# i3drobotics/i3dr_stereo_camera-ros

Measured on AMD Instinct MI355X. Metric: stereo pairs/sec + ms/frame, 1920×1080 D=256 8-path SGM, 1/2/4/8 MI355X, higher is better.
Workload: dtype u8

## Files before the change

i3dr_stereo_camera-ros_amd/csrc/census_sgm.hip:

```cpp
#include "sgm_device.h"

#include <atomic>
#include <string>

#ifndef SGM_WPE
#define SGM_WPE 4
#endif
#ifndef SGM_WPE32
#define SGM_WPE32 4
#endif
#ifndef SGM_NT_STORE
#define SGM_NT_STORE 1
#endif
#ifndef SGM_NT_LOAD
#define SGM_NT_LOAD 1
#endif
#ifndef SGM_EXP
#define SGM_EXP 0
#endif
#if SGM_EXP != 0 && !defined(SGM_EXPERIMENT_BUILD)
#error "SGM_EXP builds give invalid results: define SGM_EXPERIMENT_BUILD as well (never in a release build)"
#endif
#ifndef SGM_LRPRIO_HW
#define SGM_LRPRIO_HW 37
#endif
#ifndef SGM_LRPRIO_DIAG
#define SGM_LRPRIO_DIAG 64
#endif
#ifndef SGM_UPWTA_PRIO
#define SGM_UPWTA_PRIO 0
#endif
#ifndef SGM_ROWS_LPL8
#define SGM_ROWS_LPL8 0
#endif
#ifndef SGM_P32
#define SGM_P32 1
#endif

#include <algorithm>
#include <cstdio>
#include <cstdlib>
#include <vector>

namespace sgm {

#define SGM_CENSUS_BIT(B)                                                              \
    asm("v_cmp_lt_u32_sdwa vcc, %1, %2 src0_sel:BYTE_" #B " src1_sel:DWORD\n\t"      \
        "v_addc_co_u32_e32 %0, vcc, %0, %0, vcc"                                       \
        : "+v"(acc) : "v"(w), "v"(c) : "vcc")
__device__ __forceinline__ void census_bit(uint32_t& acc, uint32_t w, uint32_t c, int b)
{
    switch (b) {
    case 0: SGM_CENSUS_BIT(0); break;
    case 1: SGM_CENSUS_BIT(1); break;
    case 2: SGM_CENSUS_BIT(2); break;
    default: SGM_CENSUS_BIT(3); break;
    }
}
#undef SGM_CENSUS_BIT

template <int PITCH>
__device__ __forceinline__ uint64_t census_code_lds(const uint8_t* tile, int ty, int tx)
{
    static_assert(PITCH % 4 == 0, "u32 rows");
    const uint32_t* t32 = (const uint32_t*)tile + (PITCH / 4) * ty + (tx >> 2);
    const int sb = tx & 3;
    const uint32_t c = tile[(ty + 3) * PITCH + tx + 4];
    uint32_t lo = 0, hi = 0;
#pragma unroll
    for (int dy = 6; dy >= 0; dy--) {
        const uint32_t* r = t32 + (PITCH / 4) * dy;
        const uint32_t w0 = r[0], w1 = r[1], w2 = r[2];
        const uint32_t a0 = __builtin_amdgcn_alignbyte(w1, w0, sb);
        const uint32_t a1 = __builtin_amdgcn_alignbyte(w2, w1, sb);
        const uint32_t a2 = __builtin_amdgcn_alignbyte(w2, w2, sb);
#pragma unroll
        for (int dx = 8; dx >= 0; dx--) {
            if (dy == 3 && dx == 4) continue;
            const int k = dy * 9 + dx - (dy * 9 + dx > 31 ? 1 : 0);
            const uint32_t w = dx < 4 ? a0 : dx < 8 ? a1 : a2;
            if (k >= 32) census_bit(hi, w, c, dx & 3);
            else census_bit(lo, w, c, dx & 3);
        }
    }
    return (uint64_t)lo | ((uint64_t)hi << 32);
}

__global__ __launch_bounds__(256) void k_census9x7(const uint8_t* __restrict__ L, const uint8_t* __restrict__ R,
                                                   size_t stride, int W, int H,
                                                   uint64_t* __restrict__ cL, uint64_t* __restrict__ cR)
{
    __shared__ __attribute__((aligned(16))) uint8_t tile[10 * 72];
    const uint8_t* img = blockIdx.z ? R : L;
    uint64_t* out = blockIdx.z ? cR : cL;
    const int x0 = blockIdx.x * 64, y0 = blockIdx.y * 4;
    for (int i = threadIdx.x; i < 10 * 72; i += 256) {
        int ty = i / 72, tx = i - ty * 72;
        int yy = min(max(y0 + ty - 3, 0), H - 1), xx = min(max(x0 + tx - 4, 0), W - 1);
        tile[i] = img[(size_t)yy * stride + xx];
    }
    __syncthreads();
    const int tx = threadIdx.x & 63, ty = threadIdx.x >> 6;
    const int x = x0 + tx, y = y0 + ty;
    if (x >= W || y >= H) return;
    out[(size_t)y * W + x] = census_code_lds<72>(tile, ty, tx);
}

template <int DPL>
__device__ __forceinline__ void wload(const uint8_t* src, uint32_t (&wd)[(DPL + 3) / 4])
{
    if constexpr (DPL == 2) { wd[0] = *(const uint16_t*)src; }
    else if constexpr (DPL == 4) { wd[0] = *(const uint32_t*)src; }
    else if constexpr (DPL == 8) { const uint2 v = *(const uint2*)src; wd[0] = v.x; wd[1] = v.y; }
    else {
#pragma unroll
        for (int q = 0; q < DPL / 16; q++) {
// ... 245 lines not shown
    static constexpr int NPAD = LPL >= 16 ? NSEG + NSEG / 16 + 1 : NSEG + 4 * (NSEG / 32) + 4;
    static constexpr int NTOT = NSEG + NL;
    static constexpr int NLOAD = (NTOT + kWG - 1) / kWG;
    static constexpr int BUF = NPAD + NL + kWG;
    static __device__ __forceinline__ int phys(int e) { return LPL >= 16 ? e + (e >> 4) : e + 4 * (e >> 5); }
};
template <int DPL16>
struct RowsCfg {
#if SGM_ROWS_LPL8
    static constexpr int LPL = DPL16 <= 16 ? 8 : LineCfg<DPL16>::LPL;
#else
    static constexpr int LPL = LineCfg<DPL16>::LPL;
#endif
    static constexpr int DPL = DPL16 * 16 / LPL;
    static constexpr int NL = kWG / LPL;
};

template <int DPL, int LPL>
using SegRegs = uint64_t[RowSeg<DPL, LPL>::NLOAD];
template <int DPL, int LPL>
struct SegAddr {
    uint32_t off[RowSeg<DPL, LPL>::NLOAD];
    const char* lo;
};
template <int DPL, int LPL>
__device__ __forceinline__ SegAddr<DPL, LPL> seg_addr(const uint64_t* cL, const uint64_t* cR, const Geom& g, int tid)
{
    using RS = RowSeg<DPL, LPL>;
    SegAddr<DPL, LPL> a;
    const uint64_t* base = cL < cR ? cL : cR;
    const int bias = LPL * DPL + max(g.minD, 0);
    a.lo = (const char*)base - (size_t)8 * bias;
#pragma unroll
    for (int m = 0; m < RS::NLOAD; m++) {
        const int q = min(tid + m * kWG, RS::NTOT - 1);
        const int rel = q < RS::NSEG ? (int)(cR - base) + q - g.minD - LPL * DPL + 1 : (int)(cL - base) + (q - RS::NSEG);
        a.off[m] = (uint32_t)(8 * (rel + bias));
    }
    return a;
}
template <int DPL, int LPL>
__device__ __forceinline__ void seg_load(SegRegs<DPL, LPL>& v, const SegAddr<DPL, LPL>& a,
                                         const Geom& g, int rx, int ry, int xb, int s)
{
    const int y = ry > 0 ? s : g.H - 1 - s;
    const int yc = (SGM_EXP & 1) ? 0 : min(max(y, 0), g.H - 1);
    const char* sb = a.lo + (size_t)8 * ((size_t)yc * g.W + (xb + rx * s));
#pragma unroll
    for (int m = 0; m < RowSeg<DPL, LPL>::NLOAD; m++) v[m] = *(const uint64_t*)(sb + a.off[m]);
}

template <int DPL, int LPL>
__device__ __forceinline__ void seg_store(uint64_t* buf, const SegRegs<DPL, LPL>& v, int tid)
{
    using RS = RowSeg<DPL, LPL>;
#pragma unroll
    for (int m = 0; m < RS::NLOAD; m++) {
        const int q0 = tid + m * kWG;
        const int at = q0 < RS::NSEG ? RS::phys(q0) : (q0 < RS::NTOT ? RS::NPAD + (q0 - RS::NSEG) : RS::NPAD + RS::NL + tid);
        buf[at] = v[m];
    }
}

template <int DPL, bool EXACT, int LPL>
__device__ __forceinline__ void p16_seed(const uint8_t* src, const uint32_t (&imask)[DPL / 2], uint32_t (&Lr)[DPL / 2])
{
    uint32_t wd[(DPL + 3) / 4], Labs[DPL / 2];
    wload<DPL>(src, wd);
#pragma unroll
    for (int i = 0; i < DPL / 2; i++) {
        const uint32_t pr = __builtin_amdgcn_perm(0u, wd[i / 2], (i & 1) ? 0x0c030c02u : 0x0c010c00u);
        Labs[i] = pr | kBaseP2;
        if (!EXACT) Labs[i] = pk_max(Labs[i], imask[i]);
    }
    p16_relative<DPL, LPL>(Labs, Lr);
}

struct UpWta {
    const uint8_t* vols;
    size_t vol_bytes;
    uint64_t* res;
};
struct WtaPix { int best, minS, d16; bool rej; };
template <int DPL, bool EXACT>
__device__ __forceinline__ WtaPix wta_pix16(const uint32_t (&E)[(DPL + 3) / 4], const uint32_t (&O)[(DPL + 3) / 4],
                                            int p, const Geom& g, float inv_u, uint32_t* srow);
template <int DPL, bool EXACT>
__device__ __forceinline__ void wta_emask(int p, const Geom& g, uint32_t (&emaskE)[(DPL + 3) / 4],
                                          uint32_t (&emaskO)[(DPL + 3) / 4]);
template <int DPL>
__host__ __device__ constexpr size_t upwta_lds_bytes() { return (size_t)8 * 2 * RowSeg<DPL, 16>::BUF + (size_t)16 * 32 * ((DPL + 3) / 4) * 4; }

template <int DPL, bool EXACT, int LPL, bool FUSE = false, bool PRIO = false, int NP = 8>
__device__ __forceinline__ void p16_rows(const uint64_t* __restrict__ cL, const uint64_t* __restrict__ cR,
                                         uint8_t* __restrict__ V, uint8_t* __restrict__ trash, const Geom& g, int dir,
                                         int xb, const PathLaunch16& pl, uint64_t* lds, const UpWta& uw = UpWta{})
{
    static_assert(!FUSE || LPL == 16, "up+WTA blocks use 16 lanes per line (the WTA layout)");
    using RS = RowSeg<DPL, LPL>;
    constexpr int M = DPL / 2;
    constexpr int NL = RS::NL;
    const int tid = threadIdx.x;
    const int lane = tid & 63, w = tid >> 6;
    const int r = lane >> 4;
    const int p = LPL == 32 ? lane & 31 : LPL == 16 ? lane & 15 : (lane & 15) >> 1;
    const int j = LPL == 32 ? 2 * w + (lane >> 5) : LPL == 16 ? 4 * w + r : 8 * w + 2 * r + (lane & 1);
    const int rx = dir_rx(dir), ry = dir_ry(dir);
    int s0, s1;
    if (rx == 0) { s0 = 0; s1 = g.H; }
    else if (rx > 0) { s0 = max(0, g.minX1 - xb - (NL - 1)); s1 = min(g.H, g.maxX1 - xb); }
    else { s0 = max(0, xb - g.maxX1 + 1); s1 = min(g.H, xb + NL - g.minX1); }
    if (s0 >= s1) return;
    uint32_t imask[M], start[M];
    make_imask<DPL, EXACT, LPL>(p, g.D, imask, start);
    const uint32_t P1P1 = (uint32_t)g.P1 * 0x10001u, P2P2 = ((uint32_t)g.P2 + kBaseP) * 0x10001u;
    uint32_t Lr[M];
#pragma unroll
    for (int i = 0; i < M; i++) Lr[i] = start[i];
    bool pv = false;
    const uint8_t* bnd = pl.bnd[ry > 0 ? 0 : 1];
    if (bnd && s0 == 0) {
        const int x = xb + j, xp = x - rx;
        const bool cont = x >= g.minX1 && x < g.maxX1 && xp >= g.minX1 && xp < g.maxX1;
        const int xs = min(max(xp, g.minX1), g.maxX1 - 1) - g.minX1;
        uint32_t Ls[M];
        p16_seed<DPL, EXACT, LPL>(bnd + bnd_slot_of(dir) * pl.bnd_slot + (size_t)xs * g.D + p * DPL, imask, Ls);
#pragma unroll
        for (int i = 0; i < M; i++) Lr[i] = cont ? Ls[i] : Lr[i];
        pv = cont;
    }
    const bool lane_act = EXACT || p * DPL < g.D;
    const bool hi_ok = EXACT || p * DPL + 16 < g.D;
    uint8_t* const tr = trash + (tid & 63) * DPL;
    const int e_hi = j + (LPL - p) * DPL - 1;

    uint64_t* buf0 = lds;
    uint64_t* buf1 = lds + RS::BUF;
    uint64_t R0[RS::NLOAD], R1[RS::NLOAD], R2[RS::NLOAD], R3[RS::NLOAD];
    const SegAddr<DPL, LPL> sa = seg_addr<DPL, LPL>(cL, cR, g, tid);
    seg_load<DPL, LPL>(R0, sa, g, rx, ry, xb, s0);
    seg_store<DPL, LPL>(buf0, R0, tid);
    seg_load<DPL, LPL>(R1, sa, g, rx, ry, xb, min(s0 + 1, s1 - 1));
    seg_load<DPL, LPL>(R2, sa, g, rx, ry, xb, min(s0 + 2, s1 - 1));
    seg_load<DPL, LPL>(R3, sa, g, rx, ry, xb, min(s0 + 3, s1 - 1));
    __syncthreads();

    constexpr int NWD = (DPL + 3) / 4;
    constexpr int NV = NP - 1;
    uint32_t vw[NV][NWD], emaskE[NWD], emaskO[NWD];
    uint32_t* srow = (uint32_t*)(lds + 2 * RS::BUF) + j * 32 * NWD;
    const float inv_u = 1.0f / (float)max(100 - g.uniq, 1);
    const uint32_t voff = (uint32_t)((min(max(xb + j, g.minX1), g.maxX1 - 1) - g.minX1) * g.D + (lane_act ? p * DPL : 0));
    uint64_t vols0 = (uint64_t)uw.vols;
    if constexpr (FUSE) asm volatile("" : "+s"(vols0));
    auto vload = [&](int s) {
        const uint8_t* rb = (const uint8_t*)vols0 + (size_t)max(g.H - 1 - s, 0) * g.width1 * g.D;
#pragma unroll
        for (int k = 0; k < NV; k++) wload_buf<DPL>(rb + (size_t)(k == 0 ? 0 : k + 1) * uw.vol_bytes, voff, vw[k]);
    };
    if constexpr (FUSE) {
        wta_emask<DPL, EXACT>(p, g, emaskE, emaskO);
        vload(s0);
    }
    const uint64_t* resrow = FUSE ? uw.res + (size_t)(g.H - 1 - s0) * g.W : nullptr;
    auto step = [&](int s, const uint64_t* bufc) {
        const int x = xb + j + rx * s;
        const bool valid = s < s1 && x >= g.minX1 && x < g.maxX1;
        const int y = ry > 0 ? s : g.H - 1 - s;
        const uint64_t cl = bufc[RS::NPAD + j];
        uint32_t Labs[M];
        uint32_t E[NWD], O[NWD];
        if constexpr (FUSE) {
#pragma unroll
            for (int jj = 0; jj < NWD; jj++) {
                uint32_t e = 0, o = 0;
#pragma unroll
                for (int k = 0; k < NV; k++) {
                    e += vw[k][jj] & 0x00FF00FFu;
                    o += __builtin_amdgcn_perm(0u, vw[k][jj], 0x0c030c01u);
                }
                asm("" : "+v"(e), "+v"(o));
                E[jj] = e;
                O[jj] = o;
            }
        }
        const uint32_t P2x = pv ? P2P2 : kBaseP2;
        if constexpr (FUSE) __builtin_amdgcn_sched_barrier(0);
        p16_step<DPL, EXACT, LPL>(Lr, cl, [&](int k) { return bufc[RS::phys(e_hi - k)]; }, P1P1, P2x, imask, Labs);
        if constexpr (FUSE) {
            __builtin_amdgcn_sched_barrier(0);
#pragma unroll
            for (int jj = 0; jj < NWD; jj++) {
                const uint32_t a = Labs[2 * jj], b = 2 * jj + 1 < M ? Labs[2 * jj + 1] : 0u;
                E[jj] = (E[jj] + __builtin_amdgcn_perm(b, a, 0x0c040c00u)) | emaskE[jj];
                O[jj] = (O[jj] + __builtin_amdgcn_perm(b, a, 0x0c060c02u)) | emaskO[jj];
            }
            vload(s + 1);
            __builtin_amdgcn_sched_barrier(0);
            const WtaPix px = wta_pix16<DPL, EXACT>(E, O, p, g, inv_u, srow);
            const uint64_t v = (uint64_t)(uint16_t)(px.rej ? g.invalid : px.d16) |
                               ((uint64_t)(uint16_t)(px.rej ? -1 : px.best) << 16) | ((uint64_t)(uint16_t)px.minS << 32);
            const __amdgpu_buffer_rsrc_t rr = __builtin_amdgcn_make_buffer_rsrc((void*)resrow, 0, g.W * 8, 0x00020000);
            resrow -= g.W;
            typedef unsigned int v2u __attribute__((ext_vector_type(2)));
            __builtin_amdgcn_raw_buffer_store_b64(__builtin_bit_cast(v2u, v), rr,
                                                  (valid && p == 0) ? (uint32_t)x * 8u : 0x80000000u, 0, 2);
        } else {
            const bool ok = valid && lane_act && !((SGM_EXP & 2) && dir == 1);
            uint8_t* const vrow = V + (size_t)min(max(y, 0), g.H - 1) * g.width1 * g.D;
            uint8_t* const dst = ok ? vrow + (uint32_t)((x - g.minX1) * g.D + p * DPL) : tr;
            store_pairs<DPL>(dst, (ok && hi_ok) ? dst + 16 : tr + 16, Labs);
        }
        pv = valid;
    };
    auto body = [&](int s, const uint64_t* bcur, uint64_t* bnext, uint64_t (&Rnext)[RS::NLOAD],
                    uint64_t (&Rfree)[RS::NLOAD]) {
        seg_load<DPL, LPL>(Rfree, sa, g, rx, ry, xb, min(s + 4, s1 - 1));
        step(s, bcur);
        seg_store<DPL, LPL>(bnext, Rnext, tid);
        __syncthreads();
    };
    for (int s = s0; s < s1; s += 4) {
        if constexpr (PRIO) lr_prio(rx != 0 ? ((s1 - s) * SGM_LRPRIO_DIAG) >> 6 : s1 - s, g.H);
        body(s, buf0, buf1, R1, R0);
        body(s + 1, buf1, buf0, R2, R1);
        body(s + 2, buf0, buf1, R3, R2);
        body(s + 3, buf1, buf0, R0, R3);
    }
}

template <int DPL>
__host__ __device__ constexpr int rows_lds_codes() { return 2 * RowSeg<RowsCfg<DPL>::DPL, RowsCfg<DPL>::LPL>::BUF; }

template <int DPL, bool EXACT, bool PRIO = false, int NP = 0>
__device__ __forceinline__ void paths_block16(const PathFrames& pf, size_t vol_bytes, size_t trash_off,
                                              const Geom& g, const PathLaunch16& pl, uint32_t it, uint64_t* lds)
{
    using RC = RowsCfg<DPL>;
    using HC = LineCfg<DPL>;
    const int dir = (int)(it >> 24);
    const int f = (int)((it >> 22) & 3u);
    const int lb = (int)(it & 0x3FFFFFu);
    if (f >= pf.n || ((pf.skip_dirs >> dir) & 1u)) return;
    const uint64_t* cL = pick4(pf.cL, f);
    const uint64_t* cR = pick4(pf.cR, f);
    uint8_t* V = pick4(pf.vols, f) + (size_t)vol_slot(NP ? NP : pf.np, dir) * vol_bytes;
    uint8_t* trash = V + trash_off;
    const int y0 = lb * HC::HROWS + (64 / HC::LPL) * (threadIdx.x >> 6);
    if (dir == 6) p16_horiz<HC::DPL, EXACT, 1, PRIO, HC::LPL>(cL, cR, V, trash, g, y0);
    else if (dir == 7) p16_horiz<HC::DPL, EXACT, -1, PRIO, HC::LPL>(cL, cR, V, trash, g, y0);
    else p16_rows<RC::DPL, EXACT, RC::LPL, false, PRIO>(cL, cR, V, trash, g, dir, pl.xb_lo[dir] + lb * RC::NL, pl, lds);
}

__device__ __forceinline__ void trace_record(uint64_t* trace, uint64_t tag, uint64_t t0)
{
    const uint64_t t1 = __builtin_amdgcn_s_memrealtime();
    const uint32_t hw = __builtin_amdgcn_s_getreg((4 << 0) | (0 << 6) | (31 << 11));
    const uint32_t xcc = __builtin_amdgcn_s_getreg((20 << 0) | (0 << 6) | (15 << 11));
    uint64_t* r = trace + ((size_t)blockIdx.x * 4 + (threadIdx.x >> 6)) * 4;
    r[0] = tag | ((uint64_t)blockIdx.x << 32); r[1] = ((uint64_t)xcc << 32) | hw; r[2] = t0; r[3] = t1;
}

template <int DPL, bool EXACT>
__global__ __launch_bounds__(kWG) __attribute__((amdgpu_waves_per_eu(DPL >= 32 && !SGM_P32 ? SGM_WPE32 : SGM_WPE)))
void k_census_paths16(PathFrames pf, size_t vol_bytes, size_t trash_off, Geom g, PathLaunch16 pl,
                      const uint32_t* __restrict__ items, uint64_t* __restrict__ trace)
{
    __shared__ uint64_t lds[rows_lds_codes<DPL>()];
    const uint64_t t0 = trace ? __builtin_amdgcn_s_memrealtime() : 0;
    paths_block16<DPL, EXACT, true>(pf, vol_bytes, trash_off, g, pl, items[blockIdx.x], lds);
    if (trace && (threadIdx.x & 63) == 0)
        trace_record(trace, items[blockIdx.x], t0);
}

template <int DPL>
__host__ __device__ constexpr size_t wta_key_bytes(int W)
{
    return (size_t)kWG * 8 * ((DPL + 3) / 4) > (size_t)4 * W ? (size_t)kWG * 8 * ((DPL + 3) / 4) : (size_t)4 * W;
}
template <int DPL>
__host__ __device__ constexpr size_t wta_lds_bytes(int W) { return wta_key_bytes<DPL>(W) + RowLds::rest_bytes(W); }

template <int DPL, bool EXACT>
__device__ __forceinline__ WtaPix wta_pix16(const uint32_t (&E)[(DPL + 3) / 4], const uint32_t (&O)[(DPL + 3) / 4],
                                            int p, const Geom& g, float inv_u, uint32_t* srow)
{
    constexpr int NWD = (DPL + 3) / 4;
    constexpr int KB = DPL > 16 ? 5 : 4;
    constexpr uint32_t KMASK = (1u << KB) - 1;
    constexpr int G = pair_group(DPL);
    auto kof = [](int b) { return (uint32_t)(b < DPL ? vol_byte_d(G, b) : b) & KMASK; };
    uint32_t km = 0xFFFFFFFFu;
#pragma unroll
    for (int j = 0; j < NWD; j++) {
        uint32_t ce = (kof(4 * j + 2) << 16) | kof(4 * j), co = (kof(4 * j + 3) << 16) | kof(4 * j + 1);
        uint32_t ke, ko;
        if constexpr (EXACT && DPL >= 4) {
            asm("" : "+s"(ce), "+s"(co));
            ke = (E[j] << KB) | ce; ko = (O[j] << KB) | co;
        }
        else { ke = pk_shl(E[j], KB) | ce; ko = pk_shl(O[j], KB) | co; }
        km = pk_min(km, pk_min(ke, ko));
    }
    km = pk_min(km, alignbit16(km, km)) & 0xFFFFu;
    const uint32_t kmin = row_min_u32(((km >> KB) << 9) | (uint32_t)(p * DPL + (int)(km & KMASK)));
    WtaPix r;
    const int best = (int)(kmin & 511u);
    const int minS = (int)(kmin >> 9);
#pragma unroll
    for (int j = 0; j < NWD; j++) { srow[p * 2 * NWD + j] = E[j]; srow[p * 2 * NWD + NWD + j] = O[j]; }
    auto s_at = [&](int d) {
        const int kk = vol_d_byte(G, d % DPL);
        const uint32_t v = srow[(d / DPL) * 2 * NWD + (kk & 1) * NWD + (kk >> 2)];
        return (int)((v >> (16 * ((kk >> 1) & 1))) & 0xFFFFu);
    };
    const int sm = s_at(max(best - 1, 0)), sp = s_at(min(best + 1, 16 * DPL - 1));
    int T = 0;
    if (g.uniq < 100) {
        if (minS > 0) {
            const int num = minS * 100 - 1, den = 100 - g.uniq;
            int q = (int)((float)num * inv_u);
            q += (q + 1) * den <= num ? 1 : 0;
            q -= q * den > num ? 1 : 0;
            T = min(q + 1, 8 * 255 + 1);
        }
    } else {
        T = (minS == 0 && g.uniq > 100) ? 1 : 0;
    }
    const uint32_t TT = (uint32_t)T * 0x10001u;
    uint32_t acc = 0;
#pragma unroll
    for (int j = 0; j < NWD; j++) acc += pk_subs(TT, E[j]) + pk_subs(TT, O[j]);
    const int tot = (int)row_sum_u32(__builtin_amdgcn_sad_u16(acc, 0u, 0u));
    const int win = max(T - minS, 0) + (best > 0 ? max(T - sm, 0) : 0) + (best < g.D - 1 ? max(T - sp, 0) : 0);
    int outside = tot - win;
    if (g.uniq >= 100) {
        const int nwin = 1 + (best > 0 ? 1 : 0) + (best < g.D - 1 ? 1 : 0);
        outside = minS > 0 ? g.D - nwin : (g.uniq > 100 ? (g.D - nwin) - outside : 0);
    }
    r.rej = outside > 0;
    const int den = max(sm + sp - 2 * minS, 1);
    const bool use = g.subpix && best > 0 && best < g.D - 1;
    r.d16 = best * 16 + (use ? tdiv_rcp((sm - sp) * 16 + den, 2 * den) : 0) + g.minD * 16;
    r.best = best;
    r.minS = minS;
    return r;
}

template <int DPL, bool EXACT>
__device__ __forceinline__ void wta_emask(int p, const Geom& g, uint32_t (&emaskE)[(DPL + 3) / 4],
                                          uint32_t (&emaskO)[(DPL + 3) / 4])
{
#pragma unroll
    for (int j = 0; j < (DPL + 3) / 4; j++) {
        auto bad = [&](int b) { return b >= DPL || (!EXACT && p * DPL + vol_byte_d(pair_group(DPL), b) >= g.D); };
        emaskE[j] = (bad(4 * j) ? 0xFFFFu : 0u) | (bad(4 * j + 2) ? 0xFFFF0000u : 0u);
        emaskO[j] = (bad(4 * j + 1) ? 0xFFFFu : 0u) | (bad(4 * j + 3) ? 0xFFFF0000u : 0u);
    }
}

template <int DPL, bool EXACT, int NP, typename OutT = int16_t>
__device__ __forceinline__ void wta_row16(const uint8_t* __restrict__ vols, size_t vol_bytes, const Geom& g,
                                          OutT* __restrict__ out, size_t out_stride, int y, uint32_t* lds)
{
    constexpr int NWD = (DPL + 3) / 4;
    uint32_t* sl = lds;
    RowLds R(lds, (char*)lds + wta_key_bytes<DPL>(g.W), g.W);
    const int tid = threadIdx.x, lane = tid & 63;
    const int w = __builtin_amdgcn_readfirstlane(tid >> 6);
    const int r = lane >> 4, p = lane & 15;
    R.init(g, tid, kWG, false);
    const bool lane_act = EXACT || p * DPL < g.D;
    const size_t row0 = (size_t)y * g.width1 * g.D;
    const uint32_t off0 = (uint32_t)(lane_act ? p * DPL : 0);
    uint32_t* srow = sl + (w * 4 + r) * 32 * NWD;
    uint32_t emaskE[NWD], emaskO[NWD];
    wta_emask<DPL, EXACT>(p, g, emaskE, emaskO);
    const float inv_u = 1.0f / (float)max(100 - g.uniq, 1);
    const int n = g.width1;
    const int nq = (n + 3) / 4;
    const uint32_t loff = off0 + (uint32_t)(r * g.D);
    auto load = [&](int q, uint32_t (&v)[NP][NWD]) {
        const uint8_t* rowq = vols + row0 + (size_t)(4 * q) * g.D;
#pragma unroll
        for (int vv = 0; vv < NP; vv++) {
            if ((SGM_EXP & 4) && vv == 1) { for (int j = 0; j < NWD; j++) v[vv][j] = 0; continue; }
            wload_buf<DPL>(rowq + (size_t)vv * vol_bytes, loff, v[vv]);
        }
    };
    uint32_t E[NWD], O[NWD];
    auto sum8 = [&](const uint32_t (&v)[NP][NWD]) {
#pragma unroll
        for (int j = 0; j < NWD; j++) {
            uint32_t e = 0, o = 0;
#pragma unroll
            for (int vv = 0; vv < NP; vv++) {
                e += v[vv][j] & 0x00FF00FFu;
                o += __builtin_amdgcn_perm(0u, v[vv][j], 0x0c030c01u);
            }
            E[j] = e | emaskE[j];
            O[j] = o | emaskO[j];
        }
    };
    uint32_t nxt[NP][NWD];
    load(min(w, nq - 1), nxt);
    sum8(nxt);
    for (int q = w; q < nq; q += 4) {
        load(min(q + 4, nq - 1), nxt);
        const WtaPix px = wta_pix16<DPL, EXACT>(E, O, p, g, inv_u, srow);
        const int x1 = 4 * q + r;
        const bool wr = p == 0 && x1 < n;
        const int x = wr ? g.minX1 + x1 : g.W + lane;
        R.bst[x] = (int16_t)(px.rej ? -1 : px.best);
        R.mins[x] = (uint16_t)px.minS;
        R.drow[(wr && !px.rej) ? x : g.W + lane] = (int16_t)px.d16;
        sum8(nxt);
    }
    R.init_key(g, tid, kWG);
    row_finish(g, tid, kWG, R.drow, R.bst, R.mins, R.key, (int16_t*)R.mins, out + (size_t)y * out_stride);
}

template <int DPL, bool EXACT, int NP>
__device__ __forceinline__ void wta_block16(const WtaFrames& wf, size_t vol_bytes, const Geom& g, size_t out_stride,
                                            int b, uint32_t* lds)
{
    const int f = b / g.H;
    wta_row16<DPL, EXACT, NP>(pick4(wf.vols, f), vol_bytes, g, pick4(wf.out, f), out_stride, b - f * g.H, lds);
}

// ... 365 lines not shown
```

i3dr_stereo_camera-ros_amd/csrc/sgm_api.cpp:

```cpp
#include <hip/hip_runtime.h>

#include <algorithm>
#include <chrono>
#include <condition_variable>
#include <cstdio>
#include <cstdlib>
#include <cstring>
#include <functional>
#include <mutex>
#include <string>
#include <thread>
#include <vector>

#include "sgm_device.h"
#include "sgm_hip.h"

namespace sgm {
hipError_t launch_census(const uint8_t*, const uint8_t*, size_t, int, int, uint64_t*, uint64_t*, hipStream_t);
int census_path_items(const Geom&, unsigned, int, int, uint32_t*, int, int up_group = 0);
int census_vol_group(int D);
hipError_t launch_census_paths(const PathFrames&, size_t, const Geom&, const uint32_t*, int, hipStream_t,
                               const uint8_t* = nullptr, const uint8_t* = nullptr, size_t = 0);
hipError_t launch_census_wta(const WtaFrames&, size_t, const Geom&, size_t, hipStream_t, int np = 8);
hipError_t launch_rectify_map(const double*, const double*, const double*, int, int, float*, float*, size_t,
// ... 101 lines not shown
    g = Geom{};
    g.W = W; g.H = H;
    g.minD = p.min_disparity; g.D = p.num_disparities;
    const int maxD = g.minD + g.D;
    if (p.mode == SGM_MODE_CENSUS8) {
        g.P1 = p.p1 > 0 ? p.p1 : 10;
        g.P2 = std::max(p.p2 > 0 ? p.p2 : 120, g.P1 + 1);
        if (g.P2 > 193) g.P2 = 193;
        if (g.P1 >= g.P2) g.P1 = g.P2 - 1;
        g.subpix = p.subpixel != 0; g.lr = p.lr_check != 0;
        g.SW2 = 4; g.SH2 = 3; g.ftzero = 0;
    } else {
        const int sw = p.block_size > 0 ? p.block_size : 5;
        g.SW2 = sw / 2; g.SH2 = sw / 2;
        g.ftzero = std::max(p.prefilter_cap, 15) | 1;
        g.P1 = p.p1 > 0 ? p.p1 : 2;
        g.P2 = std::max(p.p2 > 0 ? p.p2 : 5, g.P1 + 1);
        g.subpix = 1; g.lr = 1;
        g.compat = p.ocv_compat & (SGM_OCV_COL0_LEGACY | SGM_OCV_SIMD_SAT | SGM_OCV_LANE_TIE);
        const bool sat = (g.compat & SGM_OCV_SIMD_SAT) != 0;
        g.ovf_thr = sat ? 32767 - g.P2 : 32767;
        const long long cmax = (long long)(2 * g.SW2 + 1) * (2 * g.SH2 + 1) * (2 * g.ftzero + 63) + g.P2 +
                               (sat ? g.P2 : 0);
        const char* wide_env = std::getenv("SGM_OCV_WIDE");
        const char* gate_env = std::getenv("SGM_OCV_GATE");
        if (wide_env && std::atoi(wide_env) != 0) g.wide = 1;
        else if (cmax > 32767) g.wide = (gate_env && std::atoi(gate_env) == 0) ? 1 : 2;
        else g.wide = 0;
    }
    g.uniq = p.uniqueness_ratio >= 0 ? p.uniqueness_ratio : 10;
    g.disp12 = p.disp12_max_diff > 0 ? p.disp12_max_diff : 1;
    g.minX1 = std::max(maxD, 0);
    g.maxX1 = W + std::min(g.minD, 0);
    g.width1 = g.maxX1 - g.minX1;
    g.invalid = (g.minD - 1) * 16;
    return SGM_OK;
}

bool use_median(const sgm_params& p)
{
    if (p.mode == SGM_MODE_OCV_BM) return false;
    return p.mode != SGM_MODE_CENSUS8 || p.median != 0;
}

bool use_speckle(const sgm_params& p)
{
    return p.speckle_window_size > 0 && (p.mode != SGM_MODE_OCV_BM || p.speckle_range >= 0);
}

struct Workspace {
    void* base = nullptr;
    size_t size = 0;
};

}

struct sgm_handle {
    int device = 0;
    sgm_params params{};
    sgm_bm_params bm = kBmDefaults;
    int census_paths = 8;
    hipStream_t stream = nullptr;
    std::string err;
    std::mutex mu;
    Workspace ws;
    uint8_t* pin = nullptr;
    size_t pin_size = 0;
    bool profiling = false;
    std::vector<hipEvent_t> ev_pool;
    size_t ev_used = 0;
    struct LaunchRec { int stage; size_t ev0, ev1; };
    std::vector<LaunchRec> launches;
    int prof_frames = 0;
    int nstages = 0;
    const char* stage_name[SGM_MAX_STAGES] = {};
    double stage_bytes[SGM_MAX_STAGES] = {};
    std::vector<sgm_handle*> sub;
    int n_cu = 0;
    int* aux = nullptr;
    size_t aux_n = 0;
    uint32_t* items_pin = nullptr;
    int items_cap = 0;
    std::string items_key[2];
    int16_t* cubic_tab = nullptr;
    bool rect_on = false;
    sgm::RectifyIn rect{};
    std::vector<sgm_handle*> bands;
    std::vector<sgm_handle*> par;
    hipEvent_t par_ev = nullptr;
    hipStream_t stream2 = nullptr;
    hipEvent_t bev[4] = {};
    hipEvent_t done = nullptr;
    hipStream_t done_stream = nullptr;
    void* io_dev = nullptr;
    size_t io_dev_size = 0;
    uint8_t* io_pin = nullptr;
    size_t io_pin_size = 0;
    hipStream_t up = nullptr, down = nullptr;
    std::vector<hipEvent_t> io_ev;
    struct HostReg { char* host; size_t bytes; char* dev; };
    std::vector<HostReg> regs;
    hipStream_t cpy = nullptr;
    hipEvent_t cpy_ev = nullptr;
};

namespace {

int fail(sgm_handle* h, int code, const std::string& msg)
{
    if (h) h->err = msg;
    return code;
}

int hip_fail(sgm_handle* h, hipError_t e, const char* where)
{
    return fail(h, SGM_ERR_DEVICE, std::string(where) + ": " + hipGetErrorString(e));
}

#define HIP_TRY(expr, where)                                   \
    do {                                                       \
        hipError_t e_ = (expr);                                \
        if (e_ != hipSuccess) return hip_fail(h, e_, where);   \
    } while (0)

int ensure_stream(sgm_handle* h)
{
    HIP_TRY(hipSetDevice(h->device), "hipSetDevice");
    if (!h->stream) HIP_TRY(hipStreamCreateWithFlags(&h->stream, hipStreamNonBlocking), "hipStreamCreate");
    if (!h->done) HIP_TRY(hipEventCreateWithFlags(&h->done, hipEventDisableTiming), "hipEventCreate");
    if (!h->n_cu) HIP_TRY(hipDeviceGetAttribute(&h->n_cu, hipDeviceAttributeMultiprocessorCount, h->device), "attr");
    return SGM_OK;
}

int order_after_last(sgm_handle* h, hipStream_t st)
{
    if (h->done_stream && h->done_stream != st) HIP_TRY(hipStreamWaitEvent(st, h->done, 0), "hipStreamWaitEvent");
    return SGM_OK;
}

int mark_done(sgm_handle* h, hipStream_t st)
{
    HIP_TRY(hipEventRecord(h->done, st), "hipEventRecord");
    h->done_stream = st;
    return SGM_OK;
}

long record_event(sgm_handle* h)
{
    if (h->ev_used == h->ev_pool.size()) {
        hipEvent_t e;
        if (hipEventCreate(&e) != hipSuccess) return -1;
        h->ev_pool.push_back(e);
    }
    if (hipEventRecord(h->ev_pool[h->ev_used], h->stream) != hipSuccess) return -1;
    return (long)h->ev_used++;
}

int stage_index(sgm_handle* h, const char* name, double bytes)
{
    for (int i = 0; i < h->nstages; i++)
        if (std::strcmp(h->stage_name[i], name) == 0) { h->stage_bytes[i] = bytes; return i; }
    if (h->nstages == SGM_MAX_STAGES) return -1;
    h->stage_name[h->nstages] = name;
    h->stage_bytes[h->nstages] = bytes;
    return h->nstages++;
}
// ... 369 lines not shown
            cf.rectL[f] = rectLs ? rectLs[k * G + f] : nullptr;
            cf.rectR[f] = rectRs ? rectRs[k * G + f] : nullptr;
        }
        return cf;
    };
    auto hk_in = [&](int k) { return hooks ? hooks->inputs(k * G, frames_of(k)) : 0; };
    auto hk_free = [&](int k) { return hooks ? hooks->outputs_free(k * G, frames_of(k)) : 0; };
    auto hk_done = [&](int k) { return hooks ? hooks->outputs_done(k * G, frames_of(k)) : 0; };
    int hrc = hk_in(0);
    if (hrc) return hrc;
    if (h->rect_on) {
        rec.begin("rectify+census", (2 * WH + 16 * WH + 16 * WH) * frames_of(0));
        HIP_TRY(sgm::launch_census_tiles(census_frames(0), g.W, g.H, st), "rectify+census");
    } else {
        for (int f = 0; f < frames_of(0); f++) {
            rec.begin("census", 2 * WH + 16 * WH);
            HIP_TRY(sgm::launch_census(dLs[f], dRs[f], stride, g.W, g.H, (uint64_t*)(ws + l.cL[code_set(0, f)]),
                                       (uint64_t*)(ws + l.cR[code_set(0, f)]), st), "census");
        }
    }
    for (int k = 0; k <= ng; k++) {
        if (k + 1 < ng && ng > 1 && (hrc = hk_in(k + 1))) return hrc;
        if (k > 0 && (hrc = hk_free(k - 1))) return hrc;
        if (up && k < ng) {
            const bool last = k == ng - 1;
            sgm::PathFrames pf = path_frames(k);
            pf.skip_dirs = last ? 0u : 2u;
            const sgm::WtaFrames wf = k > 0 ? wta_frames(k - 1) : sgm::WtaFrames{};
            const sgm::CensusFrames cf = k + 1 < ng ? census_frames(k + 1) : sgm::CensusFrames{};
            const char* name8 = last ? (wf.n ? "paths8+up_wta" : "paths8")
                                     : (wf.n ? (cf.n ? "paths7+up_wta+census" : "paths7+up_wta")
                                             : (cf.n ? "paths7+census" : "paths7"));
            const char* name4 = last ? (wf.n ? "paths4+up_wta" : "paths4")
                                     : (wf.n ? (cf.n ? "paths3+up_wta+census" : "paths3+up_wta")
                                             : (cf.n ? "paths3+census" : "paths3"));
            rec.begin(np == 4 ? name4 : name8,
                      (last ? np : np - 1) * cells * pf.n + ((np + 1) * cells + 2 * WH) * wf.n + 18 * WH * cf.n);
            HIP_TRY(sgm::launch_census_fused(pf, wf, cf, l.vol_bytes, g, items, n_items, dst_stride, true, st),
                    "fused");
            if (wf.n) {
                rec.begin("rowfin", 10 * WH * wf.n);
                HIP_TRY(sgm::launch_census_rowfin(wf, g, dst_stride, st), "rowfin");
            }
        } else if (k == ng) {
            rec.begin("wta_lr", (np * cells + 2 * WH) * frames_of(k - 1));
            HIP_TRY(sgm::launch_census_wta(wta_frames(k - 1), l.vol_bytes, g, dst_stride, st, np), "wta");
        } else if (ng == 1) {
            rec.begin(np == 4 ? "paths4" : "paths8", np * cells * frames_of(0));
            HIP_TRY(sgm::launch_census_paths(path_frames(0), l.vol_bytes, g, items, n_items, st), "paths");
        } else {
            const sgm::WtaFrames wf = k > 0 ? wta_frames(k - 1) : sgm::WtaFrames{};
            const sgm::CensusFrames cf = k + 1 < ng ? census_frames(k + 1) : sgm::CensusFrames{};
            const char* name8 = wf.n ? (cf.n ? "paths8+wta_lr+census" : "paths8+wta_lr") : "paths8+census";
            const char* name4 = wf.n ? (cf.n ? "paths4+wta_lr+census" : "paths4+wta_lr") : "paths4+census";
            rec.begin(np == 4 ? name4 : name8,
                      np * cells * frames_of(k) + (np * cells + 2 * WH) * wf.n + 18 * WH * cf.n);
            HIP_TRY(sgm::launch_census_fused(path_frames(k), wf, cf, l.vol_bytes, g, items, n_items, dst_stride, false,
                                             st),
                    "fused");
        }
        if (k > 0) {
            const int k1 = k - 1;
            for (int f = 0; f < frames_of(k1); f++) {
                int rc = run_post(h, l, g, outs[k1 * G + f], out_stride, rec, (size_t)f * g.W * g.H);
                if (rc) return rc;
            }
            if ((hrc = hk_done(k1))) return hrc;
        }
    }
    rec.end();
    return SGM_OK;
}

int prepare(sgm_handle* h, int W, int H, bool host_io, Geom& g, Layout& l, int group = 0)
{
    int rc = make_geom(h->params, W, H, g, h->err, &h->bm);
    if (rc) return rc;
    if (h->params.mode == SGM_MODE_CENSUS8 && h->census_paths != 4 && h->census_paths != 8)
        return fail(h, SGM_ERR_PARAM, "census paths must be 4 or 8 (sgm_set_census_paths), got " +
                                          std::to_string(h->census_paths));
    if ((rc = ensure_stream(h))) return rc;
    l = make_layout(h->params, g, host_io, group, h->n_cu, h->census_paths);
    if (h->params.mode != SGM_MODE_CENSUS8) { h->items_key[0].clear(); h->items_key[1].clear(); }
    return ensure_ws(h, l.total);
}

int ocv_batch_lanes(int n)
{
    const char* e = std::getenv("SGM_OCV_STREAMS");
    const int s = e ? std::atoi(e) : 4;
    return std::max(1, std::min({s, n, 8}));
}

int run_batch_ocv(sgm_handle* h, const Layout& l0, const Geom& g0, int W, int H, const uint8_t* const* dLs,
                  const uint8_t* const* dRs, int n, size_t stride, int16_t* const* outs, size_t out_stride)
{
    const int Smax = ocv_batch_lanes(n);
    size_t free_b = 0, total_b = 0;
    HIP_TRY(hipMemGetInfo(&free_b, &total_b), "hipMemGetInfo");
    const size_t reserve = std::max<size_t>(total_b / 64, (size_t)1 << 30);
    std::vector<Geom> g(1, g0);
    std::vector<Layout> l(1, l0);
    while ((int)h->par.size() < Smax - 1) h->par.push_back(nullptr);
    int S = 1;
    for (int s = 1; s < Smax; s++) {
        sgm_handle*& q = h->par[s - 1];
        const size_t have = q ? q->ws.size : 0;
        const size_t extra = have >= l0.total ? 0 : l0.total;
        if (extra + reserve > free_b) break;
        if (!q && sgm_create(&q, h->device) != SGM_OK) break;
        q->params = h->params;
        q->bm = h->bm;
        q->census_paths = h->census_paths;
        Geom gq;
        Layout lq;
        if (prepare(q, W, H, false, gq, lq) != SGM_OK) {
            q->err.clear();
            break;
        }
        free_b -= std::min(free_b, extra);
        g.push_back(gq);
        l.push_back(lq);
        S = s + 1;
    }
    if (S > 1) {
        if (!h->par_ev) HIP_TRY(hipEventCreateWithFlags(&h->par_ev, hipEventDisableTiming), "hipEventCreate");
        HIP_TRY(hipEventRecord(h->par_ev, h->stream), "hipEventRecord");
        for (int s = 1; s < S; s++) HIP_TRY(hipStreamWaitEvent(h->par[s - 1]->stream, h->par_ev, 0), "hipStreamWaitEvent");
    }
    for (int i = 0; i < n; i++) {
        const int s = i % S;
        sgm_handle* q = s ? h->par[s - 1] : h;
        const int rc = run_pipeline(q, l[s], g[s], dLs[i], dRs[i], stride, outs[i], out_stride);
        if (rc) return q == h ? rc : fail(h, rc, q->err);
    }
    for (int s = 1; s < S; s++) {
        sgm_handle* q = h->par[s - 1];
        HIP_TRY(hipEventRecord(q->done, q->stream), "hipEventRecord");
        q->done_stream = q->stream;
        HIP_TRY(hipStreamWaitEvent(h->stream, q->done, 0), "hipStreamWaitEvent");
    }
    const char* keep = std::getenv("SGM_OCV_KEEP_LANES");
    if ((size_t)(S - 1) * l0.total > total_b / 4 && !(keep && std::atoi(keep))) {
        for (int s = 1; s < S; s++) {
            sgm_handle* q = h->par[s - 1];
            HIP_TRY(hipStreamSynchronize(q->stream), "hipStreamSynchronize");
            HIP_TRY(hipFree(q->ws.base), "hipFree lane workspace");
            q->ws = Workspace{};
            q->items_key[0].clear();
            q->items_key[1].clear();
        }
    }
    return SGM_OK;
}

int match_host(sgm_handle* h, const uint8_t* L, const uint8_t* R, int W, int H, size_t stride, void* out,
               size_t out_stride, bool f32)
{
    Geom g;
    Layout l;
    int rc = prepare(h, W, H, true, g, l);
    if (rc || (rc = order_after_last(h, h->stream))) return rc;
    hipStream_t st = h->stream;
    const size_t es = f32 ? 4 : 2;
    char* ws = (char*)h->ws.base;
    const sgm_params& p = h->params;
// ... 1464 lines not shown
```

Baseline: 748.7.

## Defer fused up-path WTA finish and result stores to batched 16-row flushes

```diff
diff --git a/i3dr_stereo_camera-ros_amd/csrc/census_sgm.hip b/i3dr_stereo_camera-ros_amd/csrc/census_sgm.hip
--- a/i3dr_stereo_camera-ros_amd/csrc/census_sgm.hip
+++ b/i3dr_stereo_camera-ros_amd/csrc/census_sgm.hip
@@ -32,6 +32,12 @@
 #endif
 #ifndef SGM_ROWS_LPL8
 #define SGM_ROWS_LPL8 0
+#endif
+#ifndef SGM_UPWTA_DEFER
+#define SGM_UPWTA_DEFER 1
+#endif
+#ifndef SGM_UPWTA_SHSUM
+#define SGM_UPWTA_SHSUM 0
 #endif
 #ifndef SGM_P32
 #define SGM_P32 1
@@ -443,6 +449,11 @@
     uint64_t* res;
 };
 struct WtaPix { int best, minS, d16; bool rej; };
+struct WtaScan { int best, minS, sm, sp, T, tot; };
+template <int DPL, bool EXACT>
+__device__ __forceinline__ WtaScan wta_scan16(const uint32_t (&E)[(DPL + 3) / 4], const uint32_t (&O)[(DPL + 3) / 4],
+                                              int p, const Geom& g, float inv_u, uint32_t* srow);
+__device__ __forceinline__ WtaPix wta_finish(const WtaScan& sc, const Geom& g);
 template <int DPL, bool EXACT>
 __device__ __forceinline__ WtaPix wta_pix16(const uint32_t (&E)[(DPL + 3) / 4], const uint32_t (&O)[(DPL + 3) / 4],
                                             int p, const Geom& g, float inv_u, uint32_t* srow);
@@ -450,7 +461,10 @@
 __device__ __forceinline__ void wta_emask(int p, const Geom& g, uint32_t (&emaskE)[(DPL + 3) / 4],
                                           uint32_t (&emaskO)[(DPL + 3) / 4]);
 template <int DPL>
-__host__ __device__ constexpr size_t upwta_lds_bytes() { return (size_t)8 * 2 * RowSeg<DPL, 16>::BUF + (size_t)16 * 32 * ((DPL + 3) / 4) * 4; }
+__host__ __device__ constexpr size_t upwta_lds_bytes()
+{
+    return (size_t)8 * 2 * RowSeg<DPL, 16>::BUF + (size_t)16 * 32 * ((DPL + 3) / 4) * 4 + (SGM_UPWTA_DEFER ? 16 * 16 * 16 : 0);
+}
 
 template <int DPL, bool EXACT, int LPL, bool FUSE = false, bool PRIO = false, int NP = 8>
 __device__ __forceinline__ void p16_rows(const uint64_t* __restrict__ cL, const uint64_t* __restrict__ cR,
@@ -509,7 +523,8 @@
     constexpr int NWD = (DPL + 3) / 4;
     constexpr int NV = NP - 1;
     uint32_t vw[NV][NWD], emaskE[NWD], emaskO[NWD];
-    uint32_t* srow = (uint32_t*)(lds + 2 * RS::BUF) + j * 32 * NWD;
+    constexpr int SROW = 32 * NWD + (SGM_UPWTA_DEFER ? 64 : 0);
+    uint32_t* srow = (uint32_t*)(lds + 2 * RS::BUF) + j * SROW;
     const float inv_u = 1.0f / (float)max(100 - g.uniq, 1);
     const uint32_t voff = (uint32_t)((min(max(xb + j, g.minX1), g.maxX1 - 1) - g.minX1) * g.D + (lane_act ? p * DPL : 0));
     uint64_t vols0 = (uint64_t)uw.vols;
@@ -523,7 +538,30 @@
         wta_emask<DPL, EXACT>(p, g, emaskE, emaskO);
         vload(s0);
     }
+#if SGM_UPWTA_DEFER
+    typedef uint32_t u32x4 __attribute__((ext_vector_type(4)));
+    u32x4* const latch = (u32x4*)(srow + 32 * NWD);
+    auto upwta_flush = [&](int base) {
+        int t = tid;
+        asm volatile("" : "+v"(t));
+        const int pf = t & 15, x = xb + (t >> 4);
+        const u32x4 lt = ((const u32x4*)((uint32_t*)(lds + 2 * RS::BUF) + (t >> 4) * SROW + 32 * NWD))[pf];
+        const WtaScan sc{(int)(lt.x & 0xFFFFu), (int)(lt.x >> 16), (int)(lt.y & 0xFFFFu), (int)(lt.y >> 16),
+                         (int)lt.z, (int)lt.w};
+        const WtaPix px = wta_finish(sc, g);
+        const uint64_t v = (uint64_t)(uint16_t)(px.rej ? g.invalid : px.d16) |
+                           ((uint64_t)(uint16_t)(px.rej ? -1 : px.best) << 16) | ((uint64_t)(uint16_t)px.minS << 32);
+        const int sl = base + pf;
+        const bool ok = sl < s1 && x >= g.minX1 && x < g.maxX1;
+        const uint64_t* row0 = uw.res + (ptrdiff_t)(g.H - 16 - base) * g.W;
+        const __amdgpu_buffer_rsrc_t rr = __builtin_amdgcn_make_buffer_rsrc((void*)row0, 0, 16 * g.W * 8, 0x00020000);
+        typedef unsigned int v2u __attribute__((ext_vector_type(2)));
+        __builtin_amdgcn_raw_buffer_store_b64(__builtin_bit_cast(v2u, v), rr,
+                                              ok ? (uint32_t)((15 - pf) * g.W + x) * 8u : 0x80000000u, 0, 2);
+    };
+#else
     const uint64_t* resrow = FUSE ? uw.res + (size_t)(g.H - 1 - s0) * g.W : nullptr;
+#endif
     auto step = [&](int s, const uint64_t* bufc) {
         const int x = xb + j + rx * s;
         const bool valid = s < s1 && x >= g.minX1 && x < g.maxX1;
@@ -535,11 +573,20 @@
 #pragma unroll
             for (int jj = 0; jj < NWD; jj++) {
                 uint32_t e = 0, o = 0;
+#if SGM_UPWTA_SHSUM
+#pragma unroll
+                for (int k = 0; k < NV; k++) {
+                    e += vw[k][jj] & 0x00FF00FFu;
+                    o += vw[k][jj] >> 8;
+                }
+                o -= (e >> 16) << 8;
+#else
 #pragma unroll
                 for (int k = 0; k < NV; k++) {
                     e += vw[k][jj] & 0x00FF00FFu;
                     o += __builtin_amdgcn_perm(0u, vw[k][jj], 0x0c030c01u);
                 }
+#endif
                 asm("" : "+v"(e), "+v"(o));
                 E[jj] = e;
                 O[jj] = o;
@@ -558,6 +605,11 @@
             }
             vload(s + 1);
             __builtin_amdgcn_sched_barrier(0);
+#if SGM_UPWTA_DEFER
+            const WtaScan sc = wta_scan16<DPL, EXACT>(E, O, p, g, inv_u, srow);
+            latch[(s - s0) & 15] = u32x4{(uint32_t)sc.best | ((uint32_t)sc.minS << 16),
+                                         (uint32_t)sc.sm | ((uint32_t)sc.sp << 16), (uint32_t)sc.T, (uint32_t)sc.tot};
+#else
             const WtaPix px = wta_pix16<DPL, EXACT>(E, O, p, g, inv_u, srow);
             const uint64_t v = (uint64_t)(uint16_t)(px.rej ? g.invalid : px.d16) |
                                ((uint64_t)(uint16_t)(px.rej ? -1 : px.best) << 16) | ((uint64_t)(uint16_t)px.minS << 32);
@@ -566,6 +618,7 @@
             typedef unsigned int v2u __attribute__((ext_vector_type(2)));
             __builtin_amdgcn_raw_buffer_store_b64(__builtin_bit_cast(v2u, v), rr,
                                                   (valid && p == 0) ? (uint32_t)x * 8u : 0x80000000u, 0, 2);
+#endif
         } else {
             const bool ok = valid && lane_act && !((SGM_EXP & 2) && dir == 1);
             uint8_t* const vrow = V + (size_t)min(max(y, 0), g.H - 1) * g.width1 * g.D;
@@ -587,7 +640,17 @@
         body(s + 1, buf1, buf0, R2, R1);
         body(s + 2, buf0, buf1, R3, R2);
         body(s + 3, buf1, buf0, R0, R3);
-    }
+#if SGM_UPWTA_DEFER
+        if constexpr (FUSE)
+            if (((s - s0) & 12) == 12) upwta_flush(s - 12);
+#endif
+    }
+#if SGM_UPWTA_DEFER
+    if constexpr (FUSE) {
+        const int done = (s1 - s0 + 3) & ~3;
+        if (done & 15) upwta_flush(s0 + (done & ~15));
+    }
+#endif
 }
 
 template <int DPL>
@@ -643,8 +706,8 @@
 __host__ __device__ constexpr size_t wta_lds_bytes(int W) { return wta_key_bytes<DPL>(W) + RowLds::rest_bytes(W); }
 
 template <int DPL, bool EXACT>
-__device__ __forceinline__ WtaPix wta_pix16(const uint32_t (&E)[(DPL + 3) / 4], const uint32_t (&O)[(DPL + 3) / 4],
-                                            int p, const Geom& g, float inv_u, uint32_t* srow)
+__device__ __forceinline__ WtaScan wta_scan16(const uint32_t (&E)[(DPL + 3) / 4], const uint32_t (&O)[(DPL + 3) / 4],
+                                              int p, const Geom& g, float inv_u, uint32_t* srow)
 {
     constexpr int NWD = (DPL + 3) / 4;
     constexpr int KB = DPL > 16 ? 5 : 4;
@@ -665,7 +728,6 @@
     }
     km = pk_min(km, alignbit16(km, km)) & 0xFFFFu;
     const uint32_t kmin = row_min_u32(((km >> KB) << 9) | (uint32_t)(p * DPL + (int)(km & KMASK)));
-    WtaPix r;
     const int best = (int)(kmin & 511u);
     const int minS = (int)(kmin >> 9);
 #pragma unroll
@@ -693,6 +755,13 @@
 #pragma unroll
     for (int j = 0; j < NWD; j++) acc += pk_subs(TT, E[j]) + pk_subs(TT, O[j]);
     const int tot = (int)row_sum_u32(__builtin_amdgcn_sad_u16(acc, 0u, 0u));
+    return WtaScan{best, minS, sm, sp, T, tot};
+}
+
+__device__ __forceinline__ WtaPix wta_finish(const WtaScan& sc, const Geom& g)
+{
+    const int best = sc.best, minS = sc.minS, sm = sc.sm, sp = sc.sp, T = sc.T, tot = sc.tot;
+    WtaPix r;
     const int win = max(T - minS, 0) + (best > 0 ? max(T - sm, 0) : 0) + (best < g.D - 1 ? max(T - sp, 0) : 0);
     int outside = tot - win;
     if (g.uniq >= 100) {
@@ -706,6 +775,12 @@
     r.best = best;
     r.minS = minS;
     return r;
+}
+template <int DPL, bool EXACT>
+__device__ __forceinline__ WtaPix wta_pix16(const uint32_t (&E)[(DPL + 3) / 4], const uint32_t (&O)[(DPL + 3) / 4],
+                                            int p, const Geom& g, float inv_u, uint32_t* srow)
+{
+    return wta_finish(wta_scan16<DPL, EXACT>(E, O, p, g, inv_u, srow), g);
 }
 
 template <int DPL, bool EXACT>
diff --git a/i3dr_stereo_camera-ros_amd/csrc/sgm_api.cpp b/i3dr_stereo_camera-ros_amd/csrc/sgm_api.cpp
--- a/i3dr_stereo_camera-ros_amd/csrc/sgm_api.cpp
+++ b/i3dr_stereo_camera-ros_amd/csrc/sgm_api.cpp
@@ -207,6 +207,7 @@
     uint32_t* items_pin = nullptr;
     int items_cap = 0;
     std::string items_key[2];
+    std::string layout_sig;
     int16_t* cubic_tab = nullptr;
     bool rect_on = false;
     sgm::RectifyIn rect{};
@@ -742,6 +743,13 @@
     if ((rc = ensure_stream(h))) return rc;
     l = make_layout(h->params, g, host_io, group, h->n_cu, h->census_paths);
     if (h->params.mode != SGM_MODE_CENSUS8) { h->items_key[0].clear(); h->items_key[1].clear(); }
+    char sig[128];
+    snprintf(sig, sizeof sig, "%d %d %d %d %d %d %zu %zu", g.W, g.H, g.D, g.minD, group, l.np, l.items[0], l.items[1]);
+    if (h->layout_sig != sig) {
+        h->items_key[0].clear();
+        h->items_key[1].clear();
+        h->layout_sig = sig;
+    }
     return ensure_ws(h, l.total);
 }
 
```

Result: no change. 754.1, median of 2 (+0.7%).
